# imperatormk/candle-birefnet

Hardware: AMD Instinct MI355X
Metric: images/sec @1024x1024 Swin-L (higher is better)
Workload: dtype f32 storage+accumulate; GEMM operands as two fp16 planes of the power-of-two-scaled operand (22-bit mantissa), 3 fp16 MFMAs/product (fp32-equivalent inside the fp16 range: |GEMM input| < 8190); 1 GPU; BASELINE configs[1]: Swin-L 1024x1024 batch=1 fp32 on 1xMI355X (single-image latency); batch_per_gpu=1, global_batch=1, size=1024, deform_mode=reference_cpu, compute=f32_half2, streams_per_gpu=1, branch_streams_per_gpu=5, inputs=resident in HBM (torch cuda tensors), weights: synthetic seed 42

## Files before the change

candle_birefnet_amd/csrc/brn_graph.cpp:

```cpp
#include "brn_graph.h"

namespace brn {

float* Arena::alloc(size_t nfloats) {
    const size_t bytes = (nfloats * sizeof(float) + 255) & ~(size_t)255;
    const size_t off = top;
    top += bytes;
    if (top > peak) peak = top;
    if (dry) return reinterpret_cast<float*>(off);
    if (top > cap) fail(BRN_ERR_OOM, "workspace arena overflow: need %zu bytes, have %zu", top, cap);
    return reinterpret_cast<float*>(base + off);
}

Map new_map(Ctx& c, int B, int H, int W, int C) { return Map(c.act_alloc((size_t)B * H * W * C), B, H, W, C); }

const Switches& switches() {
    static const Switches sw = [] {
        Switches v;
#define BRN_X(field, name, dflt, doc) if (const char* e = getenv(name)) v.field = atoi(e);
        BRN_SWITCHES(BRN_X)
#undef BRN_X
        return v;
    }();
    return sw;
}

static int conv_out_size(int in, int k, const GemmW& w) { return (in + 2 * w.pad - w.dil * (k - 1) - 1) / w.stride + 1; }
static void fill_geometry(GemmParams& p, const GemmW& w, int Hin, int Win, int Cin, int Hout, int Wout) {
    p.Hin = Hin; p.Win = Win; p.Cin = Cin; p.kh = w.kh; p.kw = w.kw; p.stride = w.stride; p.pad = w.pad; p.dil = w.dil;
    p.Hout = Hout; p.Wout = Wout; p.Kreal = w.Kreal;
}
static void fill_epilogue(GemmParams& p, const GemmW& w) { p.bias = w.bias; p.scale = w.scale; p.shift = w.shift; p.act = w.act; }
static void fill_weights_f32(GemmParams& p, const GemmW& w) {
    p.W = w.w; p.Wp = w.wp; p.planes = w.planes; p.wp_rows = w.wp_rows;
    p.h2 = w.half;
    if (w.half) { p.a_scale = half2_act_scale(); p.out_scale = 1.f / (p.a_scale * w.w_scale); }
}
static GemmParams dense_params(const GemmW& w, const GemmIO& io) {
    GemmParams p{};
    p.A = io.A; p.C = io.C; p.M = io.M; p.N = w.N; p.K = w.K; p.mode = GEMM_DENSE; p.lda = io.lda;
    fill_epilogue(p, w);
    p.bbias = io.bbias; p.bbias_rows = io.bbias_rows;
    p.R = io.R; p.ldr = io.ldr; p.r_coff = io.r_coff; p.ldc = io.ldc; p.c_coff = io.c_coff;
    return p;
}
static GemmParams conv_params(const GemmW& w, const float* A, int Hin, int Win, int Cin, const Map& out, int Hout, int Wout) {
    GemmParams p{};
    p.A = A; p.C = out.p; p.M = out.B * Hout * Wout; p.N = w.N; p.K = w.K; p.mode = w.mode;
    fill_geometry(p, w, Hin, Win, Cin, Hout, Wout);
    fill_epilogue(p, w);
    p.bbias_rows = 1; p.ldc = out.ld; p.c_coff = out.coff;
    return p;
}
// ... 180 lines not shown
```

candle_birefnet_amd/csrc/brn_graph.h:

```cpp
#pragma once
#include "brn_host.h"
#include <cmath>
#include <cstdio>
#include <cstdlib>
#include <utility>

namespace brn {

struct Cost { double flop, bytes; };
struct Bracket {
    Ctx& c; bool on;
    Bracket(Ctx& c_, int fam, double flop, double bytes, int M = 0, int N = 0, int K = 0) : c(c_), on(c_.profile && !c_.dry) {
        if (!on) return;
        auto next = [&]() -> hipEvent_t {
            if (*c.event_next >= c.event_pool->size()) { hipEvent_t e; BRN_HIP(hipEventCreate(&e)); c.event_pool->push_back(e); }
            return (*c.event_pool)[(*c.event_next)++];
        };
        LaunchRecord r; r.fam = fam; r.flop = flop; r.bytes = bytes; r.e0 = next(); r.e1 = next(); r.M = M; r.N = N; r.K = K; r.region = c.region;
        BRN_HIP(hipEventRecord(r.e0, c.stream));
        c.records->push_back(r);
    }
    Bracket(Ctx& c_, int fam, Cost cost, int M, int N, int K) : Bracket(c_, fam, cost.flop, cost.bytes, M, N, K) {}
    ~Bracket() { if (on) (void)hipEventRecord(c.records->back().e1, c.stream); }
};
// ... 15 lines not shown
    ~Branch() {
        if (!on) return;
        (void)hipEventRecord(c.br->join_ev[k], c.stream);
        c.stream = main;
        c.pending |= 1u << k;
    }
};
inline void join_branches(Ctx& c, unsigned mask) {
    for (int k = 0; k < BRN_AUX_STREAMS; ++k)
        if (c.pending & mask & (1u << k)) BRN_HIP(hipStreamWaitEvent(c.stream, c.br->join_ev[k], 0));
    c.pending &= ~mask;
}
using WindowGenericRoute = void (*)(Ctx& c, const SwinBlockW& blk, const float* qkv, float* att, int B, int H, int W, int C, int window, int shift);
extern WindowGenericRoute g_window_generic_route;

constexpr int AUX_IPT = 3, AUX_LAT = 4;
constexpr unsigned AUX_ASPP_MASK = 7u;
struct ArenaHold { Arena& a; explicit ArenaHold(Arena& a_) : a(a_) { ++a.hold; } ~ArenaHold() { --a.hold; } };

}
```

candle_birefnet_amd/csrc/brn_graph_swin.cpp:

```cpp
#include "brn_graph.h"

namespace brn {

WindowGenericRoute g_window_generic_route = nullptr;

void swin_stage_dims(int H, int W, int patch, int hs[4], int ws[4]) {
    int h = (H + patch - 1) / patch, w = (W + patch - 1) / patch;
    for (int i = 0; i < 4; ++i) {
        hs[i] = h; ws[i] = w;
        h = (h + 1) / 2; w = (w + 1) / 2;
    }
}

static bool swin_attention_multi(Ctx& c, const SwinBlockW& blk, const float* xn, int B, int nin, const int* hs, const int* wsz, int C, int shift, float* y,
                                 const float* residual, int p2 = 0, int window = 12, const LNW* ln2 = nullptr, float* xn2 = nullptr, int ld_xn2 = 0) {
    const size_t mk = c.arena->mark();
    int M = 0;
    for (int k = 0; k < nin; ++k) M += B * hs[k] * wsz[k];
    float* qkv = c.act_alloc((size_t)M * 3 * C);
    const int ldp = p2 ? C * p2 / 2 : C;
    float* att = c.act_alloc((size_t)M * ldp);
    run_gemm(c, blk.qkv, GemmIO(xn, M, ldp).to(qkv, 3 * C).planes(p2, 0));
    if (window != 12 && window != 7) {
        if (p2) fail(BRN_ERR_INVALID_ARG, "window_size %d: the generic window route takes no plane layout", window);
// ... 18 lines not shown
            p.planes = (!c.bf16 && window == 12 && (blk.qkv.planes == 2 || blk.qkv.planes == 1)) ? blk.qkv.planes : 0;
            p.h2 = (p.planes == 2 && blk.qkv.half && switches().h2_att) ? 1 : 0;
            if (blk.qkv.half && !p.h2) p.planes = 0;
            p.pack_q = switches().att_pack_q;
            p.out_planes = p2;
            p.out_h2 = (p2 == 2 && blk.qkv.half) ? c.h2_scale : 0.f;
            nwin += (double)B * (p.Hp / window) * (p.Wp / window) * blk.heads;
            off += (size_t)B * hs[k] * wsz[k];
        }
        const double ntok = (double)window * window;
        Bracket b(c, FAM_ATTENTION, nwin * 2.0 * 2.0 * ntok * ntok * 32, (double)c.esz() * ((double)M * 4 * C), M, C, shift);
        BRN_LAUNCH(launch_window_attention2(ps[0], nin > 1 ? &ps[1] : nullptr, c.stream));
    }
    bool ln_done = false;
    if (ln2 && xn2 && !p2 && y == residual) ln_done = linear_residual_ln(c, blk.proj, att, M, ldp, y, *ln2, xn2, ld_xn2);
    if (!ln_done) run_gemm(c, blk.proj, GemmIO(att, M, ldp).to(y, C).add(residual, C).planes(p2, 0).f32(c.bf16, c.bf16));
    c.arena->release(mk);
    return ln_done;
}

void swin_attention(Ctx& c, const SwinBlockW& blk, const float* xn, int B, int H, int W, int C, int shift, float* y, const float* residual, int window) {
    swin_attention_multi(c, blk, xn, B, 1, &H, &W, C, shift, y, residual, 0, window);
}

void swin_forward_multi(Ctx& c, const SwinW& w, const SwinIn* ins, int nin, int B, bool outs_f32) {
    if (nin < 1 || nin > 2) fail(BRN_ERR_INVALID_ARG, "swin_forward_multi: 1 or 2 inputs");
    int hs[2][4], wsz[2][4];
    for (int k = 0; k < nin; ++k) swin_stage_dims(ins[k].H, ins[k].W, w.patch, hs[k], wsz[k]);
    auto rows = [&](int k, int i) { return B * hs[k][i] * wsz[k][i]; };
    auto total = [&](int i) { int m = 0; for (int k = 0; k < nin; ++k) m += rows(k, i); return m; };
// ... 21 lines not shown
                                                 xn0 ? c.at(xn0, off * E) : nullptr, E, c.bf16 == 2));
            }
            off += rows(k, 0);
        }
    } else {
        const size_t mk = c.arena->mark();
        float* t = c.arena->alloc((size_t)total(0) * E);
        size_t off = 0;
        for (int k = 0; k < nin; ++k) {
            run_conv_nchw(c, w.patch_proj, ins[k].img, B, ins[k].H, ins[k].W, Map(t + off * E, B, hs[k][0], wsz[k][0], E), true);
            off += rows(k, 0);
        }
        run_layernorm(c, w.patch_norm, t, total(0), E, LnOut(x, E));
        c.arena->release(mk);
    }
    for (int i = 0; i < 4; ++i) {
        const SwinStageW& st = w.stages[i];
        const int C = st.C, M = total(i);
        int hh[2], ww[2];
        for (int k = 0; k < nin; ++k) { hh[k] = hs[k][i]; ww[k] = wsz[k][i]; }
        float* xnext = nullptr;
        if (st.has_down) xnext = c.arena->alloc((size_t)total(i + 1) * 2 * C);
        const size_t mk = c.arena->mark();
        const int hidden = st.blocks.empty() ? 4 * C : st.blocks[0].fc1.N;
        int stage_pl = 0;
        if (!st.blocks.empty()) {
            const SwinBlockW& b0 = st.blocks[0];
            const int np = b0.qkv.planes;
#ifdef BRN_DIAG_BUILD
            const bool planes_on = switches().planes_kernel != 0;
#else
            constexpr bool planes_on = false;
#endif
            if (w.window == 12 && (np == 2 || (np == 3 && planes_on)) && b0.qkv.wp && b0.proj.wp && b0.fc1.wp && b0.fc2.wp && C % 32 == 0 && hidden % 32 == 0) stage_pl = np;
        }
        const int ldx = stage_pl ? C * stage_pl / 2 : C, ldh = stage_pl ? hidden * stage_pl / 2 : hidden;
        c.h2_scale = (stage_pl == 2 && st.blocks[0].qkv.half) ? half2_act_scale() : 0.f;
        const int yb = c.bf16;
        const bool xn_ready = i == 0 && xn0 && !stage_pl && ldx == C;
        float* xn = xn_ready ? xn0 : c.act_alloc((size_t)M * ldx);
        float* hid = c.act_alloc((size_t)M * ldh);
        for (size_t j = 0; j < st.blocks.size(); ++j) {
            const SwinBlockW& bk = st.blocks[j];
            const int shift = (j % 2 == 0) ? 0 : w.window / 2;
            const int p2 = stage_pl;
            const LnOut xn_out = LnOut(xn, ldx).planes(p2).s16(yb);
            if (!(xn_ready && j == 0)) run_layernorm(c, bk.norm1, x, M, C, xn_out);
            const bool ln2_done = swin_attention_multi(c, bk, xn, B, nin, hh, ww, C, shift, x, x, p2, w.window, &bk.norm2, xn, ldx);
            if (!ln2_done) run_layernorm(c, bk.norm2, x, M, C, xn_out);
            run_gemm(c, bk.fc1, GemmIO(xn, M, ldx).to(hid, ldh).planes(p2, p2));
            run_gemm(c, bk.fc2, GemmIO(hid, M, ldh).to(x, C).add(x, C).planes(p2, 0).f32(yb, yb));
        }
        size_t off = 0, off2 = 0;
        float* pm = nullptr;
        const int pm_pl = (st.has_down && st.reduction.wp && (st.reduction.planes == 2 || (st.reduction.planes == 3 && stage_pl == 3)) && (4 * C) % 32 == 0) ? st.reduction.planes : 0;
        const int ldpm = pm_pl ? 4 * C * pm_pl / 2 : 4 * C;
        if (st.has_down) pm = c.act_alloc((size_t)total(i + 1) * ldpm);
        for (int k = 0; k < nin; ++k) {
            const Map& o = ins[k].outs[i];
            if (o.B != B || o.H != hh[k] || o.W != ww[k] || o.C != C) fail(BRN_ERR_INVALID_ARG, "swin output window %d has the wrong shape", i);
            run_layernorm(c, st.out_norm, x + off * C, rows(k, i), C, LnOut(o).s16(outs_f32 ? 0 : yb));
            if (st.has_down) {
                const int M2 = rows(k, i + 1);
                if (!c.dry) {
                    LayerNormParams p{};
                    p.x = x + off * C; p.y = c.at(pm, off2 * ldpm); p.rows = M2; p.y_bf16 = yb; p.C = 4 * C; p.gamma = st.down_norm.g; p.beta = st.down_norm.b;
                    p.eps = 1e-5f; p.ldy = ldpm; p.y_coff = 0; p.mode = 1; p.H = hh[k]; p.W = ww[k]; p.Cin = C;
                    p.y_planes = pm_pl;
                    p.y_h2 = (pm_pl == 2 && st.reduction.half) ? half2_act_scale() : 0.f;
                    Bracket b(c, FAM_LAYERNORM, 0.0, 8.0 * M2 * 4.0 * C, M2, 4 * C, 1);
                    BRN_LAUNCH(launch_layernorm(p, c.stream));
                }
                off2 += M2;
            }
            off += rows(k, i);
        }
        if (st.has_down) run_gemm(c, st.reduction, GemmIO(pm, total(i + 1), ldpm).to(xnext, 2 * C).planes(pm_pl, 0).f32(yb, 0));
        c.h2_scale = 0.f;
        c.arena->release(mk);
        x = xnext;
    }
    c.arena->release(mk0);
}

}
```

candle_birefnet_amd/csrc/brn_host.h:

```cpp
#pragma once
#include <hip/hip_runtime.h>
#include <stdint.h>
#include <stdarg.h>
#include <string>
#include <deque>
#include <vector>
#include <unordered_map>
#include <stdexcept>
#include <mutex>
#include <type_traits>
#include "../../include/birefnet_hip.h"
#include "brn_kernels.h"

namespace brn {

struct Error : std::runtime_error {
    int code;
    Error(int c, const std::string& m) : std::runtime_error(m), code(c) {}
};
[[noreturn]] void fail(int code, const char* fmt, ...);
void set_last_error(const std::string& s);
#define BRN_HIP(call)                                                                                   \
    do {                                                                                                \
        hipError_t e_ = (call);                                                                         \
// ... 58 lines not shown
    X(split_streams,    "BRN_SPLIT_STREAMS",     2,  "sub-batch streams of a device-resident batch (at least two images per part; 1 = one stream)") \
    X(branch_streams,   "BRN_BRANCH_STREAMS",    -1, "-1 = auxiliary branch streams when the batch is one part; 0 = none; else the mask forced (7 ASPP, 8 image-patch, 16 lateral)") \
    X(cu_partition,     "BRN_CU_PARTITION",      0,  "1 / 2 = two sub-batch streams confined to half the CUs of every XCD / to four XCDs each") \
    X(wstat,            "BRN_WSTAT",             3,  "mask of the K served by gemm_wstat_bf16_kernel (1 = 192, 2 = 384)")                     \
    X(wstat_ln,         "BRN_WSTAT_LN",          1,  "0 = stage-0 projection and norm2 as two launches instead of gemm_wstat_ln_bf16_kernel")   \
    X(rowln,            "BRN_ROWLN",             0,  "mask of the widths whose projection + LayerNorm run on gemm_rowln_bf16_kernel (1 = 768, 2 = 384)") \
    X(patch_ln,         "BRN_PATCH_LN",          1,  "0 = PatchEmbed as gather GEMM + LayerNorm in the 16-bit modes too; 2 = fused without the first block's norm1") \
    X(p1_f32,           "BRN_P1_F32",            1,  "0 = the decoder's last map p1 is a 16-bit map like every other in the 16-bit modes")     \
    X(h2_att,           "BRN_H2_ATT",            1,  "0 = mode f32_half2 runs the fp32-MFMA attention kernel instead of the fp16-pair one")     \
    X(att_pack_q,       "BRN_ATT_PACK_Q",        1,  "0 = the split / bf16 attention kernels compute the pad queries too, windows in grid order; 2 = real queries only, grid order") \
    X(h2_ascale,        "BRN_H2_ASCALE",         3,  "log2 of the scale of GEMM input activations before the fp16 split of mode f32_half2 (0 .. 8)") \
    X(deform_f32,       "BRN_DEFORM_F32_KERNEL", 0,  "1 = the 16-bit modes run deformable convolutions on the fp32-MFMA gather kernel")        \
    X(planes_kernel,    "BRN_PLANES_KERNEL",     0,  "1 = split modes with P-layout A on the LDS-DMA plane kernel (diag build only)")           \
    X(conv_chunk_major, "BRN_CONV_CHUNK_MAJOR",  1,  "0 = tap-major K order of the 16-bit implicit-GEMM conv weights (read when weights are packed)") \
    X(offmod_pad8,      "BRN_OFFMOD_PAD8",       1,  "0 = the offset / modulator conv's N padded to 4 instead of 8")                         \
    X(deform_col_mb,    "BRN_DEFORM_COL_MB",     256, "MiB the column matrix of brn_deform_conv2d_offsets_forward's column route may take (never below 64 rows)")
struct Switches {
#define BRN_X(field, name, dflt, doc) int field = dflt;
    BRN_SWITCHES(BRN_X)
#undef BRN_X
};
const Switches& switches();

constexpr int BUILD_BF16 = 16;
constexpr int BUILD_HALF2 = 18;
struct WeightBuild {
    int planes = 0;
    bool f16 = false;
};

// ... 201 lines not shown
```

candle_birefnet_amd/csrc/brn_kernels.h:

```cpp
#pragma once
#include <hip/hip_runtime.h>
#include <stdint.h>

namespace brn {

enum GemmMode {
    GEMM_DENSE = 0,
    GEMM_CONV_NHWC = 1,
    GEMM_GATHER_NCHW = 2,
    GEMM_DEFORM_NHWC = 3
};
enum Act { ACT_NONE = 0, ACT_RELU = 1, ACT_GELU_ERF = 2 };

struct GemmParams {
    const float* A;
    const float* W;
    float* C;
    int M, N, K;
    int mode;
    int lda;
    int a_coff;
    int Hin, Win, Cin, kh, kw, stride, pad, dil, Hout, Wout;
    int Kreal;
    const float* om; int om_ld; int om_mask_off;
// ... 4 lines not shown
    int act;
    const float* R; int ldr; int r_coff;
    int ldc; int c_coff;
    const void* Wp; int planes; int wp_rows;
    int splitk; float* part;
    int a_planes, c_planes;
    int h2; float a_scale, out_scale;
    int wp_ld;
    int k_chunk_major;
    int c_f32, r_f32;
    int a_bf16, c_bf16;
    unsigned long long* trace;
    int abl;
};

struct GemmPlan { int cfg; int splitk; size_t ws_floats; };
GemmPlan plan_gemm(int M, int N, int K, int planes = 0);
hipError_t launch_gemm(const GemmParams& p, const GemmPlan& plan, float* ws, hipStream_t s);
inline bool gemm_split_is_ws(int cfg) { return cfg == 6 || cfg == 0 || cfg == 3 || cfg == 4 || cfg == 5; }
hipError_t launch_gemm_split(const GemmParams& p, int cfg, hipStream_t s);

int launch_cus();
void set_launch_cus(int n);
GemmPlan plan_gemm_bf16(int M, int N, int K, bool f32_residual = false, bool gelu = false);
hipError_t launch_gemm_bf16(const GemmParams& p, const GemmPlan& plan, float* ws, hipStream_t s);

bool gemm_wstat_eligible(const GemmParams& p);
hipError_t launch_gemm_wstat(const GemmParams& p, hipStream_t s);
bool patch_embed_ln_eligible(int Cin, int N, int k, int stride, int H, int W, int ldw, int ldx);
hipError_t launch_patch_embed_ln(const float* img, int B, int H, int W, const float* wgt, int ldw, const float* bias, const float* gamma,
                                 const float* beta, float eps, float* x, int ldx, hipStream_t s, const float* gamma1 = nullptr,
                                 const float* beta1 = nullptr, void* xn_bf16 = nullptr, int ldxn = 0, int xn_f16 = 0);
// ... 27 lines not shown
hipError_t launch_lds_mfma_probe(int blocks, int iters, int np, int variant, float* sink, hipStream_t s);
hipError_t launch_mfma_peak_bf16(int blocks, int iters, float* sink, unsigned long long* clk, int nacc, hipStream_t s);
hipError_t launch_mfma_peak(int blocks, int iters, float* sink, unsigned long long* clk, hipStream_t s);
#endif

struct LayerNormParams {
    const float* x; float* y;
    int rows, C;
    const float* gamma; const float* beta; float eps;
    int ldx;
    int ldy, y_coff;
    int mode; int H, W, Cin;
    int y_planes;
    float y_h2;
    int y_bf16;
};
hipError_t launch_layernorm(const LayerNormParams& p, hipStream_t s);

struct WindowAttnParams {
    const float* qkv;
    const float* qkv_bias;
    const float* rel_table;
    float* out;
    int B, H, W, C, heads;
    int Hp, Wp;
    int shift;
    float scale;
    int planes;
    int out_planes;
    int h2;
// ... 92 lines not shown
```

candle_birefnet_amd/csrc/brn_ops.cpp:

```cpp
#include "brn_api_util.h"
#include "kernels/deform_sample_geometry.h"
#include <cmath>
#include <cstring>
#include <memory>

using namespace brn;

struct brn_swin { brn_config cfg; int device; DeviceOwner own; SwinW w; std::mutex mu; int bf16 = 0; };

namespace {

thread_local WeightBuild g_op;
inline int op_s16(WeightBuild wb, bool on = true) { return on && wb.planes == BUILD_BF16 ? (wb.f16 ? 2 : 1) : 0; }
inline int attention_op_s16() { return op_s16(g_op); }

const float* round_to_s16(Ctx& c, const float* dx, size_t n, bool f16) {
    float* xb = c.arena->alloc_bytes(n * 2);
    if (!c.dry) BRN_HIP(launch_f32_to_bf16(dx, n, xb, c.stream, f16));
    return xb;
}

void through_nhwc(void* stream, int s16, const float* dx, int B, int C, int Cp, int H, int W, float* dy, int O, int Ho, int Wo,
                  const std::function<void(Ctx&, const Map&, const Map&)>& body) {
    with_arena((hipStream_t)stream, [&](Ctx& c) {
// ... 81 lines not shown
        DeviceOwner own;
        const WeightBuild wb = g_op;
        GemmW g = make_linear(own, wb, w, bias, N, K);
        LNW ln; ln.C = N; ln.g = own.upload(gamma, N); ln.b = own.upload(beta, N);
        Staging st(stream, loc);
        const float* dx = st.in(x, (size_t)M * K);
        const float* dr = st.in(residual, (size_t)M * N);
        float* dxo = st.out(x_out, (size_t)M * N);
        float* dyo = st.out(y_out, (size_t)M * N);
        const bool bf = wb.planes == BUILD_BF16;
        with_arena((hipStream_t)stream, [&](Ctx& c) {
            const float* a = bf ? round_to_s16(c, dx, (size_t)M * K, wb.f16) : dx;
            float* yb = bf ? c.arena->alloc_bytes((size_t)M * N * 2) : dyo;
            if (!c.dry) BRN_HIP(hipMemcpyAsync(dxo, dr, (size_t)M * N * sizeof(float), hipMemcpyDeviceToDevice, c.stream));
            if (!linear_residual_ln(c, g, a, M, K, dxo, ln, yb, N, true)) {
                run_gemm(c, g, GemmIO(a, M, K).to(dxo, N).add(dxo, N).f32(bf ? 1 : 0, bf ? 1 : 0));
                run_layernorm(c, ln, dxo, M, N, LnOut(yb, N).s16(bf ? 1 : 0));
            }
            if (bf && !c.dry) BRN_HIP(launch_bf16_to_f32(yb, (size_t)M * N, dyo, c.stream, wb.f16));
        }, op_s16(wb));
        st.finish();
    });
}

brn_status brn_layer_norm_forward(const float* x, int rows, int C, const float* gamma, const float* beta, float eps, float* y,
                                  brn_mem loc, int device, void* stream) {
    return guarded([&] {
        if (!x || !gamma || !beta || !y || rows < 1) fail(BRN_ERR_INVALID_ARG, "bad argument");
        if (C % 4 || C > 3072) fail(BRN_ERR_INVALID_ARG, "layer_norm width %d unsupported (multiple of 4, <= 3072)", C);
        ensure_device(device);
        DeviceOwner own;
        LNW ln; ln.C = C; ln.g = own.upload(gamma, C); ln.b = own.upload(beta, C);
// ... 373 lines not shown
```

candle_birefnet_amd/csrc/kernels/gemm_f32.hip:

```cpp
#include <cstdlib>
#include "../brn_kernels.h"
#include "gemm_common.h"

namespace brn {

constexpr int LDS_LD = 36;

template <int BM, int BN, int WM, int WN, int MODE>
__global__ void __launch_bounds__(WM* WN * 64) gemm_f32_kernel(const GemmParams p) {
    constexpr int NT = WM * WN * 64;
    constexpr int RPP = NT / 8;
    constexpr int PA = BM / RPP, PB = BN / RPP;
    constexpr int WTM = BM / WM, WTN = BN / WN, TM = WTM / 32, TN = WTN / 32;
    static_assert(PA >= 1 && PB >= 1 && TM >= 1 && TN >= 1, "tile too small for the thread count");

    constexpr int SMEM_MAIN = (BM + BN) * LDS_LD, SMEM_EPI = WM * WN * EPI_WAVE_FLOATS;
    __shared__ __attribute__((aligned(16))) float smem[SMEM_MAIN > SMEM_EPI ? SMEM_MAIN : SMEM_EPI];
    float* As = smem;
    float* Bs = smem + BM * LDS_LD;

    const int tid = threadIdx.x, lane = tid & 63, wave = tid >> 6;
    const int wm = wave / WN, wn = wave % WN;

    const TileSlice ts = tile_slice<BM, BN>(p, BK);
// ... 217 lines not shown
                if (s > 1) { pl.splitk = s; pl.ws_floats = (size_t)s * M * N; }
            }
            return pl;
        }
    }
    if (t64 < 384 && nk >= 8) {
        pl.cfg = 2;
        int s = (int)((768 + t64 - 1) / t64);
        if (s > nk / 4) s = nk / 4;
        if (s > 64) s = 64;
        if (s > 1) { pl.splitk = s; pl.ws_floats = (size_t)s * M * N; }
    }
    return pl;
}

static bool deform_on_split(const GemmParams& p) {
    return p.mode == GEMM_DEFORM_NHWC && p.planes >= 2 && p.Wp && p.om && !p.a_bf16 && !p.c_bf16 && (p.Cin % 32) == 0 && p.K == p.kh * p.kw * p.Cin &&
           ((p.lda | p.a_coff) & 3) == 0 && p.Hin + p.pad < 32768 && p.Win + p.pad < 32768 &&
           ((double)p.M / ((double)p.Hout * p.Wout) + 1.0) * p.Hin * p.Win * p.lda * 4.0 < 2147483648.0;
}
static int deform_split_plan(const GemmParams& p, int caller_slices, int& splitk) {
    const GemmPlan pp = plan_gemm(p.M, p.N, p.K, p.planes);
    splitk = pp.splitk < caller_slices ? pp.splitk : caller_slices;
    if (splitk < 1) splitk = 1;
    return gemm_split_is_ws(pp.cfg) ? 0 : 2;
}

hipError_t launch_gemm(const GemmParams& p_in, const GemmPlan& pl, float* ws, hipStream_t s) {
    if (p_in.M <= 0 || p_in.N <= 0 || p_in.K <= 0 || (p_in.K % BK) != 0) return hipErrorInvalidValue;
    if ((p_in.mode == GEMM_CONV_NHWC || p_in.mode == GEMM_DEFORM_NHWC) && (p_in.Cin % BK) != 0) return hipErrorInvalidValue;
    GemmParams p = p_in;
    p.splitk = pl.splitk < 1 ? 1 : pl.splitk;
    p.part = ws;
    if (p.splitk > 1 && !ws) return hipErrorInvalidValue;
    if (p.a_bf16 && p.mode != GEMM_DEFORM_NHWC) return hipErrorInvalidValue;
    if (p.c_bf16 && (p.splitk > 1 || p.R || (p.planes > 0 && p.Wp && p.mode != GEMM_DEFORM_NHWC && p.mode != GEMM_GATHER_NCHW))) return hipErrorInvalidValue;
    const bool deform_split = deform_on_split(p);
    int deform_cfg = 0;
    if (deform_split) deform_cfg = deform_split_plan(p, p.splitk, p.splitk);
    if (p.h2 && !(p.planes == 2 && p.Wp && (p.mode == GEMM_DENSE || p.mode == GEMM_CONV_NHWC || deform_split))) p.h2 = 0;
    if (p.h2 && !(p.a_scale > 0.f && p.out_scale > 0.f)) return hipErrorInvalidValue;
    if (p.a_planes || p.c_planes) {
        if (!(p.planes == 2 || p.planes == 3) || !p.Wp || p.mode != GEMM_DENSE || !gemm_split_is_ws(pl.cfg)) return hipErrorInvalidValue;
        if (p.a_planes && (p.a_planes != p.planes || p.lda % 16 || p.a_coff)) return hipErrorInvalidValue;
        if (p.c_planes && (p.c_planes != p.planes || p.splitk > 1 || p.R || p.N % 32 || p.ldc % 16 || p.c_coff % 32)) return hipErrorInvalidValue;
    }
    hipError_t e;
    if (p.planes > 0 && p.Wp && (p.mode == GEMM_DENSE || p.mode == GEMM_CONV_NHWC)) e = launch_gemm_split(p, pl.cfg, s);
    else if (deform_split) e = launch_gemm_split(p, deform_cfg, s);
    else if (pl.cfg == 0) e = launch_cfg<128, 128, 2, 2>(p, s);
    else if (pl.cfg == 1) e = launch_cfg<128, 64, 2, 2>(p, s);
    else if (pl.cfg == 3) e = launch_cfg<128, 128, 2, 4>(p, s);
    else if (pl.cfg == 4) e = launch_cfg<256, 128, 4, 2>(p, s);
    else if (pl.cfg == 5) e = launch_cfg<128, 128, 4, 2>(p, s);
    else e = launch_cfg<64, 64, 2, 2>(p, s);
    if (e != hipSuccess || p.splitk == 1) return e;
    long total = (long)p.M * p.N;
    long blocks = (total + 255) / 256;
    if (blocks > 4096) blocks = 4096;
    hipLaunchKernelGGL(splitk_reduce_kernel, dim3((unsigned)blocks), dim3(256), 0, s, p);
    return hipGetLastError();
}

}
```

candle_birefnet_amd/csrc/kernels/layernorm.hip:

```cpp
#include "../brn_kernels.h"
#include "split_planes.h"

namespace brn {

typedef float f32x4 __attribute__((ext_vector_type(4)));

constexpr int LN_MAX_V = 12;
constexpr int LN_WAVES = 4;

template <int MODE, int NV>
__global__ void __launch_bounds__(LN_WAVES * 64) layernorm_kernel(const LayerNormParams p) {
    const int lane = threadIdx.x & 63;
    const int nv = p.C >> 2;
    const long nwaves = (long)gridDim.x * LN_WAVES;
    for (long row = (long)blockIdx.x * LN_WAVES + (threadIdx.x >> 6); row < p.rows; row += nwaves) {
    f32x4 v[NV];
    int h2 = 0, w2 = 0, bi = 0, Ho = 0, Wo = 0;
    if (MODE == 1) {
        Ho = (p.H + 1) >> 1; Wo = (p.W + 1) >> 1;
        const int hw = Ho * Wo;
        bi = (int)(row / hw);
        const int rem = (int)(row - (long)bi * hw);
        h2 = rem / Wo; w2 = rem - h2 * Wo;
    }
    const int cin4 = p.Cin >> 2;
    float sum = 0.f;
#pragma unroll
    for (int i = 0; i < NV; ++i) {
        const int c4 = lane + i * 64;
        f32x4 t = {0.f, 0.f, 0.f, 0.f};
        if (c4 < nv) {
            if (MODE == 0) {
                t = *reinterpret_cast<const f32x4*>(p.x + row * p.ldx + c4 * 4);
            } else {
                const int part = c4 / cin4, cc = c4 - part * cin4;
                const int y = 2 * h2 + (part & 1), x = 2 * w2 + (part >> 1);
                if (y < p.H && x < p.W)
                    t = *reinterpret_cast<const f32x4*>(p.x + (((long)bi * p.H + y) * p.W + x) * p.Cin + cc * 4);
            }
            sum += (t[0] + t[1]) + (t[2] + t[3]);
        }
        v[i] = t;
    }
#pragma unroll
    for (int o = 32; o > 0; o >>= 1) sum += __shfl_xor(sum, o);
    const float mean = sum / (float)p.C;
    float sq = 0.f;
#pragma unroll
    for (int i = 0; i < NV; ++i) {
        if (lane + i * 64 < nv) {
            const f32x4 d = v[i] - mean;
            sq += (d[0] * d[0] + d[1] * d[1]) + (d[2] * d[2] + d[3] * d[3]);
        }
    }
#pragma unroll
    for (int o = 32; o > 0; o >>= 1) sq += __shfl_xor(sq, o);
    const float rstd = 1.0f / sqrtf(sq / (float)p.C + p.eps);
    float* yrow = p.y + row * p.ldy + p.y_coff;
#pragma unroll
    for (int i = 0; i < NV; ++i) {
        const int c4 = lane + i * 64;
        if (c4 < nv) {
            const f32x4 gm = *reinterpret_cast<const f32x4*>(p.gamma + c4 * 4);
            const f32x4 bt = *reinterpret_cast<const f32x4*>(p.beta + c4 * 4);
            const f32x4 o = (v[i] - mean) * rstd * gm + bt;
            if (p.y_planes && p.y_h2 > 0.f) store_planes_h(p.y + row * p.ldy, p.y_coff + c4 * 4, o, p.y_h2);
            else if (p.y_planes) store_planes_n(p.y_planes, p.y + row * p.ldy, p.y_coff + c4 * 4, o);
            else if (p.y_bf16) {
                if (p.y_bf16 == 2) {
                    typedef _Float16 f16x4_ln __attribute__((ext_vector_type(4)));
                    f16x4_ln h;
#pragma unroll
                    for (int e = 0; e < 4; ++e) h[e] = (_Float16)o[e];
                    *reinterpret_cast<f16x4_ln*>(reinterpret_cast<_Float16*>(p.y) + row * p.ldy + p.y_coff + c4 * 4) = h;
                } else {
                bf16x4 h;
#pragma unroll
                for (int e = 0; e < 4; ++e) h[e] = (__bf16)o[e];
                *reinterpret_cast<bf16x4*>(reinterpret_cast<__bf16*>(p.y) + row * p.ldy + p.y_coff + c4 * 4) = h;
                }
            } else *reinterpret_cast<f32x4*>(yrow + c4 * 4) = o;
        }
    }
    }
}

hipError_t launch_layernorm(const LayerNormParams& p, hipStream_t s) {
    if (p.C % 4 || p.C > 64 * 4 * LN_MAX_V || p.rows <= 0) return hipErrorInvalidValue;
    if (p.mode == 1 && (p.C != 4 * p.Cin || p.Cin % 4)) return hipErrorInvalidValue;
    if (p.y_bf16 && (p.y_planes || p.ldy % 4 || p.y_coff % 4)) return hipErrorInvalidValue;
    if (p.y_planes && (!(p.y_planes == 2 || p.y_planes == 3) || p.C % 32 || p.ldy % 16 || p.y_coff % 32)) return hipErrorInvalidValue;
    if (p.y_h2 > 0.f && p.y_planes != 2) return hipErrorInvalidValue;
    long blocks = (p.rows + LN_WAVES - 1) / LN_WAVES;
    if (blocks > 2048) blocks = 2048;
    dim3 grid((unsigned)blocks), block(LN_WAVES * 64);
    const int nvl = (p.C / 4 + 63) / 64;
#define BRN_LN(MODE_, NV_) hipLaunchKernelGGL((layernorm_kernel<MODE_, NV_>), grid, block, 0, s, p)
#define BRN_LN_NV(MODE_)                                                                        \
    if (nvl <= 1) BRN_LN(MODE_, 1); else if (nvl <= 2) BRN_LN(MODE_, 2); else if (nvl <= 3) BRN_LN(MODE_, 3); \
    else if (nvl <= 6) BRN_LN(MODE_, 6); else BRN_LN(MODE_, 12)
    if (p.mode == 0) { BRN_LN_NV(0); } else { BRN_LN_NV(1); }
#undef BRN_LN_NV
#undef BRN_LN
    return hipGetLastError();
}

}
```

Baseline: 97.15 images/s.

## Fuse split-K GEMM reduction with following LayerNorm in Swin blocks

```diff
diff --git a/candle_birefnet_amd/csrc/brn_gemm_ln.cpp b/candle_birefnet_amd/csrc/brn_gemm_ln.cpp
--- /dev/null
+++ b/candle_birefnet_amd/csrc/brn_gemm_ln.cpp
@@ -0,0 +1,49 @@
+#include "brn_graph.h"
+
+namespace brn {
+namespace {
+
+bool gemm_ln_route(Ctx& c, const GemmW& w, const GemmIO& io, const LNW& ln, const LnOut& out) {
+    const int sw = switches().gemm_ln;
+    if (!sw || c.bf16 || !w.wp || !(w.planes == 2 || w.planes == 3) || w.mode != GEMM_DENSE || w.act != ACT_NONE || w.scale || io.bbias || io.c_planes ||
+        out.y_s16 || ln.C != w.N || !ln.g || !ln.b || (w.N & 3) || ((io.ldc | io.c_coff) & 3) || (io.R && ((io.ldr | io.r_coff) & 3)))
+        return false;
+    const int M = io.M;
+    GemmPlan pl = plan_gemm_ln(M, w.N, w.K, w.planes);
+    if (sw == 2) {
+        pl = plan_gemm(M, w.N, w.K, w.planes);
+        pl.splitk = w.K / 32 >= 2 ? 2 : 1;
+        pl.ws_floats = (size_t)pl.splitk * M * w.N;
+        pl.raw = 1;
+    }
+    if (pl.splitk < 2) return false;
+    if (io.a_planes) pl.cfg = 0;
+    const size_t mk = c.arena->mark();
+    float* ws = c.arena->alloc(pl.ws_floats);
+    c.arena->release(mk);
+    if (c.dry) return true;
+    GemmParams p = dense_params(w, io);
+    p.bbias_rows = 1;
+    fill_weights_f32(p, w);
+    p.a_planes = io.a_planes;
+    {
+        const double mn = (double)M * w.N;
+        Bracket b(c, FAM_GEMM_DENSE, 2.0 * mn * w.K, 4.0 * ((double)M * w.K + (double)w.N * w.K + pl.splitk * mn), M, w.N, w.K);
+        BRN_LAUNCH(launch_gemm(p, pl, ws, c.stream));
+    }
+    LayerNormParams q{};
+    q.y = out.y; q.rows = M; q.C = ln.C; q.gamma = ln.g; q.beta = ln.b; q.eps = 1e-5f;
+    q.ldy = out.ldy; q.y_coff = out.y_coff; q.y_planes = out.y_planes;
+    q.y_h2 = out.y_planes == 2 ? c.h2_scale : 0.f;
+    q.part = ws; q.slices = pl.splitk; q.bias = w.bias;
+    q.R = io.R; q.ldr = io.ldr; q.r_coff = io.r_coff;
+    q.x_out = io.C; q.ldxo = io.ldc; q.xo_coff = io.c_coff;
+    Bracket b(c, FAM_LAYERNORM, 0.0, 4.0 * (pl.splitk + (io.R ? 3.0 : 2.0)) * M * (double)ln.C, M, ln.C, pl.splitk);
+    BRN_LAUNCH(launch_layernorm(q, c.stream));
+    return true;
+}
+
+struct Registrar { Registrar() { g_gemm_ln_route = &gemm_ln_route; } } registrar;
+
+}
+}
diff --git a/candle_birefnet_amd/csrc/brn_graph.cpp b/candle_birefnet_amd/csrc/brn_graph.cpp
--- a/candle_birefnet_amd/csrc/brn_graph.cpp
+++ b/candle_birefnet_amd/csrc/brn_graph.cpp
@@ -31,12 +31,12 @@
     p.Hout = Hout; p.Wout = Wout; p.Kreal = w.Kreal;
 }
 static void fill_epilogue(GemmParams& p, const GemmW& w) { p.bias = w.bias; p.scale = w.scale; p.shift = w.shift; p.act = w.act; }
-static void fill_weights_f32(GemmParams& p, const GemmW& w) {
+void fill_weights_f32(GemmParams& p, const GemmW& w) {
     p.W = w.w; p.Wp = w.wp; p.planes = w.planes; p.wp_rows = w.wp_rows;
     p.h2 = w.half;
     if (w.half) { p.a_scale = half2_act_scale(); p.out_scale = 1.f / (p.a_scale * w.w_scale); }
 }
-static GemmParams dense_params(const GemmW& w, const GemmIO& io) {
+GemmParams dense_params(const GemmW& w, const GemmIO& io) {
     GemmParams p{};
     p.A = io.A; p.C = io.C; p.M = io.M; p.N = w.N; p.K = w.K; p.mode = GEMM_DENSE; p.lda = io.lda;
     fill_epilogue(p, w);
diff --git a/candle_birefnet_amd/csrc/brn_graph.h b/candle_birefnet_amd/csrc/brn_graph.h
--- a/candle_birefnet_amd/csrc/brn_graph.h
+++ b/candle_birefnet_amd/csrc/brn_graph.h
@@ -53,6 +53,11 @@
 using WindowGenericRoute = void (*)(Ctx& c, const SwinBlockW& blk, const float* qkv, float* att, int B, int H, int W, int C, int window, int shift);
 extern WindowGenericRoute g_window_generic_route;
 
+using GemmLnRoute = bool (*)(Ctx& c, const GemmW& w, const GemmIO& io, const LNW& ln, const LnOut& out);
+extern GemmLnRoute g_gemm_ln_route;
+GemmParams dense_params(const GemmW& w, const GemmIO& io);
+void fill_weights_f32(GemmParams& p, const GemmW& w);
+
 constexpr int AUX_IPT = 3, AUX_LAT = 4;
 constexpr unsigned AUX_ASPP_MASK = 7u;
 struct ArenaHold { Arena& a; explicit ArenaHold(Arena& a_) : a(a_) { ++a.hold; } ~ArenaHold() { --a.hold; } };
diff --git a/candle_birefnet_amd/csrc/brn_graph_swin.cpp b/candle_birefnet_amd/csrc/brn_graph_swin.cpp
--- a/candle_birefnet_amd/csrc/brn_graph_swin.cpp
+++ b/candle_birefnet_amd/csrc/brn_graph_swin.cpp
@@ -3,6 +3,7 @@
 namespace brn {
 
 WindowGenericRoute g_window_generic_route = nullptr;
+GemmLnRoute g_gemm_ln_route = nullptr;
 
 void swin_stage_dims(int H, int W, int patch, int hs[4], int ws[4]) {
     int h = (H + patch - 1) / patch, w = (W + patch - 1) / patch;
@@ -56,6 +57,8 @@
     }
     bool ln_done = false;
     if (ln2 && xn2 && !p2 && y == residual) ln_done = linear_residual_ln(c, blk.proj, att, M, ldp, y, *ln2, xn2, ld_xn2);
+    if (!ln_done && ln2 && xn2 && y == residual && g_gemm_ln_route)
+        ln_done = g_gemm_ln_route(c, blk.proj, GemmIO(att, M, ldp).to(y, C).add(residual, C).planes(p2, 0).f32(c.bf16, c.bf16), *ln2, LnOut(xn2, ld_xn2).planes(p2).s16(c.bf16));
     if (!ln_done) run_gemm(c, blk.proj, GemmIO(att, M, ldp).to(y, C).add(residual, C).planes(p2, 0).f32(c.bf16, c.bf16));
     c.arena->release(mk);
     return ln_done;
@@ -107,6 +110,20 @@
         run_layernorm(c, w.patch_norm, t, total(0), E, LnOut(x, E));
         c.arena->release(mk);
     }
+    auto stage_planes = [&](const SwinStageW& sg) {
+        if (sg.blocks.empty()) return 0;
+        const SwinBlockW& b0 = sg.blocks[0];
+        const int np = b0.qkv.planes;
+#ifdef BRN_DIAG_BUILD
+        const bool planes_on = switches().planes_kernel != 0;
+#else
+        constexpr bool planes_on = false;
+#endif
+        if (w.window == 12 && (np == 2 || (np == 3 && planes_on)) && b0.qkv.wp && b0.proj.wp && b0.fc1.wp && b0.fc2.wp && sg.C % 32 == 0 && b0.fc1.N % 32 == 0) return np;
+        return 0;
+    };
+    float* xn_handoff = nullptr;
+    bool handoff_done = false;
     for (int i = 0; i < 4; ++i) {
         const SwinStageW& st = w.stages[i];
         const int C = st.C, M = total(i);
@@ -114,35 +131,36 @@
         for (int k = 0; k < nin; ++k) { hh[k] = hs[k][i]; ww[k] = wsz[k][i]; }
         float* xnext = nullptr;
         if (st.has_down) xnext = c.arena->alloc((size_t)total(i + 1) * 2 * C);
+        float* xn_made = xn_handoff;
+        xn_handoff = nullptr;
+        int next_pl = 0;
+        if (st.has_down && i + 1 < 4 && g_gemm_ln_route && !c.bf16 && !w.stages[i + 1].blocks.empty() && w.stages[i + 1].C == 2 * C) {
+            next_pl = stage_planes(w.stages[i + 1]);
+            xn_handoff = c.act_alloc((size_t)total(i + 1) * (next_pl ? 2 * C * next_pl / 2 : 2 * C));
+        }
         const size_t mk = c.arena->mark();
         const int hidden = st.blocks.empty() ? 4 * C : st.blocks[0].fc1.N;
-        int stage_pl = 0;
-        if (!st.blocks.empty()) {
-            const SwinBlockW& b0 = st.blocks[0];
-            const int np = b0.qkv.planes;
-#ifdef BRN_DIAG_BUILD
-            const bool planes_on = switches().planes_kernel != 0;
-#else
-            constexpr bool planes_on = false;
-#endif
-            if (w.window == 12 && (np == 2 || (np == 3 && planes_on)) && b0.qkv.wp && b0.proj.wp && b0.fc1.wp && b0.fc2.wp && C % 32 == 0 && hidden % 32 == 0) stage_pl = np;
-        }
+        const int stage_pl = stage_planes(st);
         const int ldx = stage_pl ? C * stage_pl / 2 : C, ldh = stage_pl ? hidden * stage_pl / 2 : hidden;
         c.h2_scale = (stage_pl == 2 && st.blocks[0].qkv.half) ? half2_act_scale() : 0.f;
         const int yb = c.bf16;
-        const bool xn_ready = i == 0 && xn0 && !stage_pl && ldx == C;
-        float* xn = xn_ready ? xn0 : c.act_alloc((size_t)M * ldx);
+        bool xn_ready = (i == 0 && xn0 && !stage_pl && ldx == C) || (xn_made && handoff_done);
+        float* xn = (i == 0 && xn_ready) ? xn0 : xn_made ? xn_made : c.act_alloc((size_t)M * ldx);
+        handoff_done = false;
         float* hid = c.act_alloc((size_t)M * ldh);
         for (size_t j = 0; j < st.blocks.size(); ++j) {
             const SwinBlockW& bk = st.blocks[j];
             const int shift = (j % 2 == 0) ? 0 : w.window / 2;
             const int p2 = stage_pl;
             const LnOut xn_out = LnOut(xn, ldx).planes(p2).s16(yb);
-            if (!(xn_ready && j == 0)) run_layernorm(c, bk.norm1, x, M, C, xn_out);
+            if (!xn_ready) run_layernorm(c, bk.norm1, x, M, C, xn_out);
+            xn_ready = false;
             const bool ln2_done = swin_attention_multi(c, bk, xn, B, nin, hh, ww, C, shift, x, x, p2, w.window, &bk.norm2, xn, ldx);
             if (!ln2_done) run_layernorm(c, bk.norm2, x, M, C, xn_out);
             run_gemm(c, bk.fc1, GemmIO(xn, M, ldx).to(hid, ldh).planes(p2, p2));
-            run_gemm(c, bk.fc2, GemmIO(hid, M, ldh).to(x, C).add(x, C).planes(p2, 0).f32(yb, yb));
+            const GemmIO fc2_io = GemmIO(hid, M, ldh).to(x, C).add(x, C).planes(p2, 0).f32(yb, yb);
+            if (j + 1 < st.blocks.size() && g_gemm_ln_route) xn_ready = g_gemm_ln_route(c, bk.fc2, fc2_io, st.blocks[j + 1].norm1, xn_out);
+            if (!xn_ready) run_gemm(c, bk.fc2, fc2_io);
         }
         size_t off = 0, off2 = 0;
         float* pm = nullptr;
@@ -168,7 +186,15 @@
             }
             off += rows(k, i);
         }
-        if (st.has_down) run_gemm(c, st.reduction, GemmIO(pm, total(i + 1), ldpm).to(xnext, 2 * C).planes(pm_pl, 0).f32(yb, 0));
+        if (st.has_down) {
+            const GemmIO red_io = GemmIO(pm, total(i + 1), ldpm).to(xnext, 2 * C).planes(pm_pl, 0).f32(yb, 0);
+            if (xn_handoff) {
+                const SwinBlockW& nb = w.stages[i + 1].blocks[0];
+                c.h2_scale = (next_pl == 2 && nb.qkv.half) ? half2_act_scale() : 0.f;
+                handoff_done = g_gemm_ln_route(c, st.reduction, red_io, nb.norm1, LnOut(xn_handoff, next_pl ? 2 * C * next_pl / 2 : 2 * C).planes(next_pl));
+            }
+            if (!handoff_done) run_gemm(c, st.reduction, red_io);
+        }
         c.h2_scale = 0.f;
         c.arena->release(mk);
         x = xnext;
diff --git a/candle_birefnet_amd/csrc/brn_host.h b/candle_birefnet_amd/csrc/brn_host.h
--- a/candle_birefnet_amd/csrc/brn_host.h
+++ b/candle_birefnet_amd/csrc/brn_host.h
@@ -96,6 +96,7 @@
     X(planes_kernel,    "BRN_PLANES_KERNEL",     0,  "1 = split modes with P-layout A on the LDS-DMA plane kernel (diag build only)")           \
     X(conv_chunk_major, "BRN_CONV_CHUNK_MAJOR",  1,  "0 = tap-major K order of the 16-bit implicit-GEMM conv weights (read when weights are packed)") \
     X(offmod_pad8,      "BRN_OFFMOD_PAD8",       1,  "0 = the offset / modulator conv's N padded to 4 instead of 8")                         \
+    X(gemm_ln,          "BRN_GEMM_LN",           1,  "split modes, GEMM -> LayerNorm with the split-K slices summed by the LayerNorm: 0 = never; 1 = where plan_gemm_ln cuts; 2 = every eligible pair, two slices") \
     X(deform_col_mb,    "BRN_DEFORM_COL_MB",     256, "MiB the column matrix of brn_deform_conv2d_offsets_forward's column route may take (never below 64 rows)")
 struct Switches {
 #define BRN_X(field, name, dflt, doc) int field = dflt;
diff --git a/candle_birefnet_amd/csrc/brn_kernels.h b/candle_birefnet_amd/csrc/brn_kernels.h
--- a/candle_birefnet_amd/csrc/brn_kernels.h
+++ b/candle_birefnet_amd/csrc/brn_kernels.h
@@ -42,8 +42,9 @@
     int abl;
 };
 
-struct GemmPlan { int cfg; int splitk; size_t ws_floats; };
+struct GemmPlan { int cfg; int splitk; size_t ws_floats; int raw = 0; };
 GemmPlan plan_gemm(int M, int N, int K, int planes = 0);
+GemmPlan plan_gemm_ln(int M, int N, int K, int planes);
 hipError_t launch_gemm(const GemmParams& p, const GemmPlan& plan, float* ws, hipStream_t s);
 inline bool gemm_split_is_ws(int cfg) { return cfg == 6 || cfg == 0 || cfg == 3 || cfg == 4 || cfg == 5; }
 hipError_t launch_gemm_split(const GemmParams& p, int cfg, hipStream_t s);
@@ -101,6 +102,10 @@
     int y_planes;
     float y_h2;
     int y_bf16;
+    const float* part; int slices;
+    const float* bias;
+    const float* R; int ldr, r_coff;
+    float* x_out; int ldxo, xo_coff;
 };
 hipError_t launch_layernorm(const LayerNormParams& p, hipStream_t s);
 
diff --git a/candle_birefnet_amd/csrc/brn_ops.cpp b/candle_birefnet_amd/csrc/brn_ops.cpp
--- a/candle_birefnet_amd/csrc/brn_ops.cpp
+++ b/candle_birefnet_amd/csrc/brn_ops.cpp
@@ -1,4 +1,5 @@
 #include "brn_api_util.h"
+#include "brn_graph.h"
 #include "kernels/deform_sample_geometry.h"
 #include <cmath>
 #include <cstring>
@@ -119,8 +120,12 @@
             float* yb = bf ? c.arena->alloc_bytes((size_t)M * N * 2) : dyo;
             if (!c.dry) BRN_HIP(hipMemcpyAsync(dxo, dr, (size_t)M * N * sizeof(float), hipMemcpyDeviceToDevice, c.stream));
             if (!linear_residual_ln(c, g, a, M, K, dxo, ln, yb, N, true)) {
-                run_gemm(c, g, GemmIO(a, M, K).to(dxo, N).add(dxo, N).f32(bf ? 1 : 0, bf ? 1 : 0));
-                run_layernorm(c, ln, dxo, M, N, LnOut(yb, N).s16(bf ? 1 : 0));
+                const GemmIO io = GemmIO(a, M, K).to(dxo, N).add(dxo, N).f32(bf ? 1 : 0, bf ? 1 : 0);
+                const LnOut yo = LnOut(yb, N).s16(bf ? 1 : 0);
+                if (!(g_gemm_ln_route && g_gemm_ln_route(c, g, io, ln, yo))) {
+                    run_gemm(c, g, io);
+                    run_layernorm(c, ln, dxo, M, N, yo);
+                }
             }
             if (bf && !c.dry) BRN_HIP(launch_bf16_to_f32(yb, (size_t)M * N, dyo, c.stream, wb.f16));
         }, op_s16(wb));
diff --git a/candle_birefnet_amd/csrc/kernels/gemm_f32.hip b/candle_birefnet_amd/csrc/kernels/gemm_f32.hip
--- a/candle_birefnet_amd/csrc/kernels/gemm_f32.hip
+++ b/candle_birefnet_amd/csrc/kernels/gemm_f32.hip
@@ -255,6 +255,17 @@
     return pl;
 }
 
+constexpr int LN_SK_MIN_KT = 48;
+GemmPlan plan_gemm_ln(int M, int N, int K, int planes) {
+    GemmPlan pl = plan_gemm(M, N, K, planes);
+    const long t128 = (long)((M + 127) / 128) * ((N + 127) / 128);
+    const double waste = (double)t128 * 128.0 * 128.0 / ((double)M * N);
+    if (planes != 2 || N < 128 || (N & 3) || waste > 1.35) { pl.splitk = 1; pl.ws_floats = 0; return pl; }
+    if (pl.splitk == 1 && t128 > 128 && t128 <= 256 && K / BK / 2 >= LN_SK_MIN_KT) { pl.splitk = 2; pl.ws_floats = (size_t)2 * M * N; }
+    pl.raw = pl.splitk > 1;
+    return pl;
+}
+
 static bool deform_on_split(const GemmParams& p) {
     return p.mode == GEMM_DEFORM_NHWC && p.planes >= 2 && p.Wp && p.om && !p.a_bf16 && !p.c_bf16 && (p.Cin % 32) == 0 && p.K == p.kh * p.kw * p.Cin &&
            ((p.lda | p.a_coff) & 3) == 0 && p.Hin + p.pad < 32768 && p.Win + p.pad < 32768 &&
@@ -281,6 +292,7 @@
     if (deform_split) deform_cfg = deform_split_plan(p, p.splitk, p.splitk);
     if (p.h2 && !(p.planes == 2 && p.Wp && (p.mode == GEMM_DENSE || p.mode == GEMM_CONV_NHWC || deform_split))) p.h2 = 0;
     if (p.h2 && !(p.a_scale > 0.f && p.out_scale > 0.f)) return hipErrorInvalidValue;
+    if (pl.raw && (p.splitk < 2 || p.c_planes || p.c_bf16)) return hipErrorInvalidValue;
     if (p.a_planes || p.c_planes) {
         if (!(p.planes == 2 || p.planes == 3) || !p.Wp || p.mode != GEMM_DENSE || !gemm_split_is_ws(pl.cfg)) return hipErrorInvalidValue;
         if (p.a_planes && (p.a_planes != p.planes || p.lda % 16 || p.a_coff)) return hipErrorInvalidValue;
@@ -295,7 +307,7 @@
     else if (pl.cfg == 4) e = launch_cfg<256, 128, 4, 2>(p, s);
     else if (pl.cfg == 5) e = launch_cfg<128, 128, 4, 2>(p, s);
     else e = launch_cfg<64, 64, 2, 2>(p, s);
-    if (e != hipSuccess || p.splitk == 1) return e;
+    if (e != hipSuccess || p.splitk == 1 || pl.raw) return e;
     long total = (long)p.M * p.N;
     long blocks = (total + 255) / 256;
     if (blocks > 4096) blocks = 4096;
diff --git a/candle_birefnet_amd/csrc/kernels/layernorm.hip b/candle_birefnet_amd/csrc/kernels/layernorm.hip
--- a/candle_birefnet_amd/csrc/kernels/layernorm.hip
+++ b/candle_birefnet_amd/csrc/kernels/layernorm.hip
@@ -1,105 +1,25 @@
-#include "../brn_kernels.h"
-#include "split_planes.h"
+#include "layernorm_row.h"
 
 namespace brn {
 
-typedef float f32x4 __attribute__((ext_vector_type(4)));
-
-constexpr int LN_MAX_V = 12;
-constexpr int LN_WAVES = 4;
-
-template <int MODE, int NV>
+template <int SRC, int NV>
 __global__ void __launch_bounds__(LN_WAVES * 64) layernorm_kernel(const LayerNormParams p) {
     const int lane = threadIdx.x & 63;
-    const int nv = p.C >> 2;
     const long nwaves = (long)gridDim.x * LN_WAVES;
-    for (long row = (long)blockIdx.x * LN_WAVES + (threadIdx.x >> 6); row < p.rows; row += nwaves) {
-    f32x4 v[NV];
-    int h2 = 0, w2 = 0, bi = 0, Ho = 0, Wo = 0;
-    if (MODE == 1) {
-        Ho = (p.H + 1) >> 1; Wo = (p.W + 1) >> 1;
-        const int hw = Ho * Wo;
-        bi = (int)(row / hw);
-        const int rem = (int)(row - (long)bi * hw);
-        h2 = rem / Wo; w2 = rem - h2 * Wo;
-    }
-    const int cin4 = p.Cin >> 2;
-    float sum = 0.f;
-#pragma unroll
-    for (int i = 0; i < NV; ++i) {
-        const int c4 = lane + i * 64;
-        f32x4 t = {0.f, 0.f, 0.f, 0.f};
-        if (c4 < nv) {
-            if (MODE == 0) {
-                t = *reinterpret_cast<const f32x4*>(p.x + row * p.ldx + c4 * 4);
-            } else {
-                const int part = c4 / cin4, cc = c4 - part * cin4;
-                const int y = 2 * h2 + (part & 1), x = 2 * w2 + (part >> 1);
-                if (y < p.H && x < p.W)
-                    t = *reinterpret_cast<const f32x4*>(p.x + (((long)bi * p.H + y) * p.W + x) * p.Cin + cc * 4);
-            }
-            sum += (t[0] + t[1]) + (t[2] + t[3]);
-        }
-        v[i] = t;
-    }
-#pragma unroll
-    for (int o = 32; o > 0; o >>= 1) sum += __shfl_xor(sum, o);
-    const float mean = sum / (float)p.C;
-    float sq = 0.f;
-#pragma unroll
-    for (int i = 0; i < NV; ++i) {
-        if (lane + i * 64 < nv) {
-            const f32x4 d = v[i] - mean;
-            sq += (d[0] * d[0] + d[1] * d[1]) + (d[2] * d[2] + d[3] * d[3]);
-        }
-    }
-#pragma unroll
-    for (int o = 32; o > 0; o >>= 1) sq += __shfl_xor(sq, o);
-    const float rstd = 1.0f / sqrtf(sq / (float)p.C + p.eps);
-    float* yrow = p.y + row * p.ldy + p.y_coff;
-#pragma unroll
-    for (int i = 0; i < NV; ++i) {
-        const int c4 = lane + i * 64;
-        if (c4 < nv) {
-            const f32x4 gm = *reinterpret_cast<const f32x4*>(p.gamma + c4 * 4);
-            const f32x4 bt = *reinterpret_cast<const f32x4*>(p.beta + c4 * 4);
-            const f32x4 o = (v[i] - mean) * rstd * gm + bt;
-            if (p.y_planes && p.y_h2 > 0.f) store_planes_h(p.y + row * p.ldy, p.y_coff + c4 * 4, o, p.y_h2);
-            else if (p.y_planes) store_planes_n(p.y_planes, p.y + row * p.ldy, p.y_coff + c4 * 4, o);
-            else if (p.y_bf16) {
-                if (p.y_bf16 == 2) {
-                    typedef _Float16 f16x4_ln __attribute__((ext_vector_type(4)));
-                    f16x4_ln h;
-#pragma unroll
-                    for (int e = 0; e < 4; ++e) h[e] = (_Float16)o[e];
-                    *reinterpret_cast<f16x4_ln*>(reinterpret_cast<_Float16*>(p.y) + row * p.ldy + p.y_coff + c4 * 4) = h;
-                } else {
-                bf16x4 h;
-#pragma unroll
-                for (int e = 0; e < 4; ++e) h[e] = (__bf16)o[e];
-                *reinterpret_cast<bf16x4*>(reinterpret_cast<__bf16*>(p.y) + row * p.ldy + p.y_coff + c4 * 4) = h;
-                }
-            } else *reinterpret_cast<f32x4*>(yrow + c4 * 4) = o;
-        }
-    }
-    }
+    for (long row = (long)blockIdx.x * LN_WAVES + (threadIdx.x >> 6); row < p.rows; row += nwaves) layernorm_row<SRC, NV>(p, row, lane);
 }
 
 hipError_t launch_layernorm(const LayerNormParams& p, hipStream_t s) {
-    if (p.C % 4 || p.C > 64 * 4 * LN_MAX_V || p.rows <= 0) return hipErrorInvalidValue;
-    if (p.mode == 1 && (p.C != 4 * p.Cin || p.Cin % 4)) return hipErrorInvalidValue;
-    if (p.y_bf16 && (p.y_planes || p.ldy % 4 || p.y_coff % 4)) return hipErrorInvalidValue;
-    if (p.y_planes && (!(p.y_planes == 2 || p.y_planes == 3) || p.C % 32 || p.ldy % 16 || p.y_coff % 32)) return hipErrorInvalidValue;
-    if (p.y_h2 > 0.f && p.y_planes != 2) return hipErrorInvalidValue;
+    if (!layernorm_params_ok(p)) return hipErrorInvalidValue;
     long blocks = (p.rows + LN_WAVES - 1) / LN_WAVES;
-    if (blocks > 2048) blocks = 2048;
+    if (blocks > LN_MAX_BLOCKS) blocks = LN_MAX_BLOCKS;
     dim3 grid((unsigned)blocks), block(LN_WAVES * 64);
-    const int nvl = (p.C / 4 + 63) / 64;
-#define BRN_LN(MODE_, NV_) hipLaunchKernelGGL((layernorm_kernel<MODE_, NV_>), grid, block, 0, s, p)
-#define BRN_LN_NV(MODE_)                                                                        \
-    if (nvl <= 1) BRN_LN(MODE_, 1); else if (nvl <= 2) BRN_LN(MODE_, 2); else if (nvl <= 3) BRN_LN(MODE_, 3); \
-    else if (nvl <= 6) BRN_LN(MODE_, 6); else BRN_LN(MODE_, 12)
-    if (p.mode == 0) { BRN_LN_NV(0); } else { BRN_LN_NV(1); }
+    const int nv = layernorm_nv(p);
+#define BRN_LN(SRC_, NV_) hipLaunchKernelGGL((layernorm_kernel<SRC_, NV_>), grid, block, 0, s, p)
+#define BRN_LN_NV(SRC_)                                                                        \
+    if (nv == 1) BRN_LN(SRC_, 1); else if (nv == 2) BRN_LN(SRC_, 2); else if (nv == 3) BRN_LN(SRC_, 3); \
+    else if (nv == 6) BRN_LN(SRC_, 6); else BRN_LN(SRC_, 12)
+    if (p.part) { BRN_LN_NV(LN_SRC_SLICES); } else if (p.mode == 0) { BRN_LN_NV(LN_SRC_ROWS); } else { BRN_LN_NV(LN_SRC_MERGE); }
 #undef BRN_LN_NV
 #undef BRN_LN
     return hipGetLastError();
diff --git a/candle_birefnet_amd/csrc/kernels/layernorm_row.h b/candle_birefnet_amd/csrc/kernels/layernorm_row.h
--- /dev/null
+++ b/candle_birefnet_amd/csrc/kernels/layernorm_row.h
@@ -0,0 +1,113 @@
+#pragma once
+#include "../brn_kernels.h"
+#include "split_planes.h"
+
+namespace brn {
+
+constexpr int LN_MAX_V = 12;
+constexpr int LN_WAVES = 4;
+constexpr int LN_MAX_BLOCKS = 2048;
+enum { LN_SRC_ROWS = 0, LN_SRC_MERGE = 1, LN_SRC_SLICES = 2 };
+
+template <int SRC, int NV>
+__device__ __forceinline__ void layernorm_row(const LayerNormParams& p, const long row, const int lane) {
+    const int nv = p.C >> 2;
+    f32x4 v[NV];
+    int h2 = 0, w2 = 0, bi = 0, Ho = 0, Wo = 0;
+    if (SRC == LN_SRC_MERGE) {
+        Ho = (p.H + 1) >> 1; Wo = (p.W + 1) >> 1;
+        const int hw = Ho * Wo;
+        bi = (int)(row / hw);
+        const int rem = (int)(row - (long)bi * hw);
+        h2 = rem / Wo; w2 = rem - h2 * Wo;
+    }
+    const int cin4 = p.Cin >> 2;
+    const long slice_stride = (long)p.rows * p.C;
+    float sum = 0.f;
+#pragma unroll
+    for (int i = 0; i < NV; ++i) {
+        const int c4 = lane + i * 64;
+        f32x4 t = {0.f, 0.f, 0.f, 0.f};
+        if (c4 < nv) {
+            if (SRC == LN_SRC_ROWS) {
+                t = *reinterpret_cast<const f32x4*>(p.x + row * p.ldx + c4 * 4);
+            } else if (SRC == LN_SRC_MERGE) {
+                const int part = c4 / cin4, cc = c4 - part * cin4;
+                const int y = 2 * h2 + (part & 1), x = 2 * w2 + (part >> 1);
+                if (y < p.H && x < p.W)
+                    t = *reinterpret_cast<const f32x4*>(p.x + (((long)bi * p.H + y) * p.W + x) * p.Cin + cc * 4);
+            } else {
+                const float* src = p.part + row * p.C + c4 * 4;
+#pragma unroll 4
+                for (int s = 0; s < p.slices; ++s) t = t + *reinterpret_cast<const f32x4*>(src + s * slice_stride);
+                if (p.bias) t = t + *reinterpret_cast<const f32x4*>(p.bias + c4 * 4);
+                if (p.R) t = t + *reinterpret_cast<const f32x4*>(p.R + row * p.ldr + p.r_coff + c4 * 4);
+            }
+            sum += (t[0] + t[1]) + (t[2] + t[3]);
+        }
+        v[i] = t;
+    }
+    if (SRC == LN_SRC_SLICES) {
+#pragma unroll
+        for (int i = 0; i < NV; ++i) {
+            const int c4 = lane + i * 64;
+            if (c4 < nv) *reinterpret_cast<f32x4*>(p.x_out + row * p.ldxo + p.xo_coff + c4 * 4) = v[i];
+        }
+    }
+#pragma unroll
+    for (int o = 32; o > 0; o >>= 1) sum += __shfl_xor(sum, o);
+    const float mean = sum / (float)p.C;
+    float sq = 0.f;
+#pragma unroll
+    for (int i = 0; i < NV; ++i) {
+        if (lane + i * 64 < nv) {
+            const f32x4 d = v[i] - mean;
+            sq += (d[0] * d[0] + d[1] * d[1]) + (d[2] * d[2] + d[3] * d[3]);
+        }
+    }
+#pragma unroll
+    for (int o = 32; o > 0; o >>= 1) sq += __shfl_xor(sq, o);
+    const float rstd = 1.0f / sqrtf(sq / (float)p.C + p.eps);
+    float* yrow = p.y + row * p.ldy + p.y_coff;
+#pragma unroll
+    for (int i = 0; i < NV; ++i) {
+        const int c4 = lane + i * 64;
+        if (c4 < nv) {
+            const f32x4 gm = *reinterpret_cast<const f32x4*>(p.gamma + c4 * 4);
+            const f32x4 bt = *reinterpret_cast<const f32x4*>(p.beta + c4 * 4);
+            const f32x4 o = (v[i] - mean) * rstd * gm + bt;
+            if (p.y_planes && p.y_h2 > 0.f) store_planes_h(p.y + row * p.ldy, p.y_coff + c4 * 4, o, p.y_h2);
+            else if (p.y_planes) store_planes_n(p.y_planes, p.y + row * p.ldy, p.y_coff + c4 * 4, o);
+            else if (p.y_bf16) {
+                if (p.y_bf16 == 2) {
+                    typedef _Float16 f16x4_ln __attribute__((ext_vector_type(4)));
+                    f16x4_ln h;
+#pragma unroll
+                    for (int e = 0; e < 4; ++e) h[e] = (_Float16)o[e];
+                    *reinterpret_cast<f16x4_ln*>(reinterpret_cast<_Float16*>(p.y) + row * p.ldy + p.y_coff + c4 * 4) = h;
+                } else {
+                bf16x4 h;
+#pragma unroll
+                for (int e = 0; e < 4; ++e) h[e] = (__bf16)o[e];
+                *reinterpret_cast<bf16x4*>(reinterpret_cast<__bf16*>(p.y) + row * p.ldy + p.y_coff + c4 * 4) = h;
+                }
+            } else *reinterpret_cast<f32x4*>(yrow + c4 * 4) = o;
+        }
+    }
+}
+
+inline bool layernorm_params_ok(const LayerNormParams& p) {
+    if (p.C % 4 || p.C > 64 * 4 * LN_MAX_V || p.rows <= 0) return false;
+    if (p.mode == 1 && (p.C != 4 * p.Cin || p.Cin % 4)) return false;
+    if (p.y_bf16 && (p.y_planes || p.ldy % 4 || p.y_coff % 4)) return false;
+    if (p.y_planes && (!(p.y_planes == 2 || p.y_planes == 3) || p.C % 32 || p.ldy % 16 || p.y_coff % 32)) return false;
+    if (p.y_h2 > 0.f && p.y_planes != 2) return false;
+    if (p.part && (p.slices < 1 || p.mode != 0 || !p.x_out || (p.ldxo | p.xo_coff) % 4 || (p.R && (p.ldr | p.r_coff) % 4))) return false;
+    return true;
+}
+inline int layernorm_nv(const LayerNormParams& p) {
+    const int nvl = (p.C / 4 + 63) / 64;
+    return nvl <= 3 ? nvl : nvl <= 6 ? 6 : 12;
+}
+
+}
```

New measurement: 98.18 images/s (median of 6 runs). +1.1%, better.
